# francescofugazzi/3dgsconverter

Measured on AMD Instinct MI355X. Metric: Msplats/sec SOR k=16, higher is better.
Workload: dtype f32 select / f64 finalize

## Files before the change

3dgsconverter_amd/_lib.py:

```python
from __future__ import annotations

import contextlib
import ctypes as C
import functools
import os
import threading
import time

import numpy as np

_HERE = os.path.dirname(os.path.abspath(__file__))
LIB_PATH = os.environ.get("GSX_LIB_PATH") or os.path.join(_HERE, "libgsx_hip.so")

KNN_AUTO, KNN_BRUTE, KNN_GRID, KNN_TREE = 0, 1, 2, 3
PROBE_ROOT_DIST2, PROBE_ROOT_DSQRT = 0, 1
PROBE_MEAN_NET, PROBE_MEAN_LIST, PROBE_MEAN_LE128, PROBE_MEAN_NP = 0, 1, 2, 3
T_SOR_KNN, T_SOR_BIN, T_SOR_FALLBACK, T_SOR_STATS, T_DENSITY, T_KMEANS_ASSIGN, T_KMEANS_UPDATE, T_QUANTIZE = range(8)
T_SLAB_PREP, T_SLAB_ROWS, T_SLAB_MEANS, T_SLAB_COLL = range(8, 12)


class GsxError(RuntimeError):
    """Raised for every failure of the HIP path (missing library, no GPU, HIP error)."""


# ... 115 lines not shown

DENSITY_OK, DENSITY_EMPTY, DENSITY_HOST = range(3)
SLAB_OK, SLAB_EMPTY, SLAB_NONFINITE, SLAB_SMALL_SHARD, SLAB_NO_STRUCTURE = range(5)
COMM_F32_MAX, COMM_F32_SUM, COMM_I64_SUM, COMM_F64_MAX, COMM_I64_MIN = range(5)

_P, _I64, _I, _D = C.c_void_p, C.c_int64, C.c_int, C.c_double
SIGNATURES = {
    "gsx_version": (C.c_char_p, []),
    "gsx_last_error": (C.c_char_p, []),
    "gsx_device_count": (_I, []),
    "gsx_device_uid": (_I, [_I, C.c_char_p, _I]),
    "gsx_ctx_create": (_I, [_I, C.POINTER(_P)]),
    "gsx_ctx_destroy": (None, [_P]),
    "gsx_ctx_set_stream": (_I, [_P, _P]),
    "gsx_ctx_own_stream": (_I, [_P]),
    "gsx_ctx_last_knn_algo": (_I, [_P]),
    "gsx_ctx_synchronize": (_I, [_P]),
    "gsx_ctx_check": (_I, [_P]),
    "gsx_ctx_set_timing": (_I, [_P, _I]),
    "gsx_ctx_reset_timing": (_I, [_P]),
    "gsx_ctx_get_timing": (_I, [_P, _I, C.POINTER(C.c_uint64), C.POINTER(_D)]),
    "gsx_ctx_set_param": (_I, [_P, C.c_char_p, _D]),
    "gsx_dev_malloc": (_I, [_P, C.c_size_t, C.POINTER(_P)]),
    "gsx_dev_free": (_I, [_P, _P]),
    "gsx_dev_upload": (_I, [_P, _P, _P, C.c_size_t]),
    "gsx_dev_download": (_I, [_P, _P, _P, C.c_size_t]),
    "gsx_dev_copy": (_I, [_P, _P, _P, C.c_size_t]),
    "gsx_dev_upload_async": (_I, [_P, _P, _P, C.c_size_t]),
    "gsx_dev_memset": (_I, [_P, _P, _I, C.c_size_t]),
    "gsx_fields_nonzero_dev": (_I, [_P, _P, _I64, _I64, _I, C.POINTER(C.c_uint64)]),
    "gsx_rows_repack_dev": (_I, [_P, _P, _I64, _I64, _P, _I64]),
    "gsx_host_pinned_alloc": (_I, [_P, C.c_size_t, C.POINTER(C.c_void_p)]),
    "gsx_host_pinned_free": (_I, [_P, _P]),
    "gsx_dev_upload_staged": (_I, [_P, _P, _P, C.c_size_t]),
    "gsx_dev_download_staged": (_I, [_P, _P, _P, C.c_size_t]),
    "gsx_host_gather_f32": (_I, [_P, _I64, _I64, C.POINTER(_I64), _I, _P]),
    "gsx_host_gather_columns_f32": (_I, [_P, _I64, _I64, C.POINTER(_I64), _I, _P]),
    "gsx_host_compact_rows": (_I, [_P, _I64, _I64, _P, _P, _I64, C.POINTER(_I64)]),
    "gsx_host_take_rows": (_I, [_P, _I64, _I64, _P, _I64, _P]),
    "gsx_host_zero_columns": (_I, [_P, _I64, _I64, C.POINTER(_I64), _I]),
    "gsx_host_append_columns": (_I, [_P, _I64, _I64, _P, _I64, _P, _I64]),
    "gsx_host_take_rows_append": (_I, [_P, _I64, _I64, _P, _I64, _P, _I64, _P, _I64]),
    "gsx_host_take_rows_shape": (_I, [_P, _I64, _I64, _P, _I64, _P, _I64, C.POINTER(_I64), _I, _P, _I64]),
    "gsx_rgb_from_sh": (_I, [_P, _I64, _P, _P]),
    "gsx_rgb_from_sh_dev": (_I, [_P, _P, _I64, _P, _P]),
    "gsx_rgb_from_sh_list": (_I, [_P, _I64, _P, _P, _I64, C.POINTER(_I64)]),
    "gsx_rgb_from_sh_list_dev": (_I, [_P, _P, _I64, _P, _P, _I64, _P]),
    "gsx_compact_rows_dev": (_I, [_P, _P, _P, _P, _I64, _P, _P, C.POINTER(_I64)]),
    "gsx_mask_bbox_dev": (_I, [_P, _P, _I64, _P, _P]),
    "gsx_mask_ge_dev": (_I, [_P, _P, _P, _I64, _D, _P]),
    "gsx_sor_knn_dev": (_I, [_P, _P, _P, _P, _I64, _I64, _I64, _I64, _I, _I, _P, C.POINTER(SorInfo)]),
    "gsx_sor_knn_share_dev": (_I, [_P, _P, _P, _P, _I64, _I64, _I, _I, _I, _I, _P, C.POINTER(SorInfo)]),
    "gsx_sor_debug_brick_plan": (_I, [_P, _P, _P, _P, _I64]),
    "gsx_sor_debug_work_queue": (_I, [_P, _P, _P, _P]),
    "gsx_sor_debug_wave_stamps": (_I, [_P, _I, _P, _I64, _P]),
    "gsx_knn_probe_root_dev": (_I, [_P, _P, _I64, _I, _P]),
    "gsx_knn_probe_mean_dev": (_I, [_P, _P, _I64, _I64, _I, _I, _I, _P]),
    "gsx_sor_stats_dev": (_I, [_P, _P, _I64, _D, _P]),
    "gsx_sor_mask_dev": (_I, [_P, _P, _I64, _P, _P]),
    "gsx_comm_unique_id": (_I, [_P]),
    "gsx_comm_init": (_I, [_P, _I, _I, _P]),
    "gsx_comm_destroy": (_I, [_P]),
    "gsx_comm_all_reduce": (_I, [_P, _P, _I64, _I]),
    "gsx_comm_all_gather": (_I, [_P, _P, _P, _I64]),
    "gsx_comm_all_to_all_v": (_I, [_P, _P, _P, _P, _P, _P, _P, _I]),
    "gsx_comm_all_to_all_segs": (_I, [_P, _P, _P, _I, _P, _P, _P, _P, _I]),
    "gsx_comm_abort": (_I, [_P]),
    "gsx_comm_transport": (_I, [_P]),
    "gsx_comm_rank": (_I, [_P, C.POINTER(_I), C.POINTER(_I)]),
    "gsx_comm_barrier": (_I, [_P]),
    "gsx_slab_plan": (_I, [_P, _I, _I, _I64, _I, _D, C.POINTER(SlabPlan)]),
    "gsx_sor_slab_step_dev": (_I, [_P, _P, _I64, _I, _D, _D, _P, C.POINTER(SlabStep)]),
    "gsx_slab_bbox_dev": (_I, [_P, _P, _P, _P, _I64, _I64, _P]),
    "gsx_slab_hist_dev": (_I, [_P, _P, _P, _P, _I64, _I64, _P, _P]),
    "gsx_slab_partition_dev": (_I, [_P, _P, _P, _P, _I64, _I64, _I, _I, C.c_float, C.c_float, _P, _I, _P, _P, _P, _P, _P]),
    "gsx_sor_knn_slab_dev": (_I, [_P, _P, _I64, _I64, _I, _P, _P]),
    "gsx_slab_certify_dev": (_I, [_P, _P, _I64, _I64, _P, C.c_float, C.c_float, _P]),
    "gsx_slab_unpermute_dev": (_I, [_P, _P, _P, _I64, _P]),
    "gsx_sor_piece_sums_dev": (_I, [_P, _P, _I64, _P, _P]),
    "gsx_sor_stats_from_pieces_dev": (_I, [_P, _P, _I64, _I64, _I, _D, _P]),
    "gsx_sor_filter": (_I, [_P, _P, _P, _I64, _I64, _I, _D, _I, _P, _P, _P, C.POINTER(SorInfo)]),
    "gsx_density_voxels": (_I, [_P, _P, _P, _I64, _I64, _D, _I64, _I64, C.POINTER(_I64), C.POINTER(_I64), _P, _P]),
    "gsx_density_mask": (_I, [_P, _P, _P, _I64, _I64, _D, _P, _I64, _P]),
    "gsx_kmeans_lloyd": (_I, [_P, _I64, _I, _I, _I, _P, _P, _P]),
    "gsx_quantize_sorted_codebook": (_I, [_P, _I64, _P, _I, _P]),
    "gsx_kmeans_pp": (_I, [_P, _I64, _I, _I, _P, _I, _P]),
    "gsx_kmeans_pp_dev": (_I, [_P, _P, _I64, _I, _I, _P, _I, _P]),
    "gsx_kmeans1d": (_I, [_P, _I64, _I, _I, _P, _P, _P]),
    "gsx_kmeans1d_dev": (_I, [_P, _P, _I64, _I, _I, _I, _P, _P, _P]),
    "gsx_lexsort3": (_I, [_P, _P, _P, _I64, _P]),
    "gsx_lexsort3_dev": (_I, [_P, _P, _P, _P, _I64, _I64, _P]),
    "gsx_sog_quats": (_I, [_P, _I64, _P]),
    "gsx_sog_positions": (_I, [_P, _I64, C.c_float, C.c_float, _P, _P]),
    "gsx_sog_positions_dev": (_I, [_P, _P, _I64, C.c_float, C.c_float, _P, _P]),
    "gsx_sog_alpha": (_I, [_P, _I64, _P, _P]),
    "gsx_sog_alpha_dev": (_I, [_P, _P, _I64, _P, _P]),
    "gsx_sog_quats_dev": (_I, [_P, _P, _I64, _P]),
    "gsx_sog_scan_dev": (_I, [_P, _P, C.POINTER(SogLayout), _I64, _P, C.POINTER(SogScan)]),
    "gsx_sog_extremes_dev": (_I, [_P, _P, _I64, _P, _P, _I, _P, _P]),
    "gsx_sog_order_dev": (_I, [_P, _P, _I64, _P]),
    "gsx_sog_gather_dev": (_I, [_P, _P, C.POINTER(SogLayout), _P, _I64, _I, _P, _P, _P, _P, _P, _P]),
    "gsx_sog_means_texels_dev": (_I, [_P, _P, _I64, _I64, _P, _P, _P, _P, _P, _P, _P, _I64, _P]),
    "gsx_sog_quats_texels_dev": (_I, [_P, _P, _I64, _I64, _P]),
    "gsx_sog_codes_texels_dev": (_I, [_P, _P, _I64, _I64, _P, _I, _P, _P, _P, _I64, _P]),
    "gsx_sog_labels_texels_dev": (_I, [_P, _P, _I64, _I64, _I64, _I, _P]),
    "gsx_gather_rows_dev": (_I, [_P, _P, _I, _P, _I64, _P]),
# ... 1853 lines not shown
        check(self.lib.gsx_ctx_synchronize(self.handle), "gsx_ctx_synchronize")

    def check(self):
        check(self.lib.gsx_ctx_check(self.handle), "gsx_ctx_check")

    def last_knn_algo(self) -> int:
        return int(self.lib.gsx_ctx_last_knn_algo(self.handle))

    def set_param(self, name: str, value: float):
        check(self.lib.gsx_ctx_set_param(self.handle, name.encode(), float(value)), "gsx_ctx_set_param")

    def set_timing(self, on: bool):
        check(self.lib.gsx_ctx_set_timing(self.handle, 1 if on else 0), "gsx_ctx_set_timing")

    def reset_timing(self):
        check(self.lib.gsx_ctx_reset_timing(self.handle), "gsx_ctx_reset_timing")

    def timing(self, slot: int):
        n = C.c_uint64()
        ms = C.c_double()
        check(self.lib.gsx_ctx_get_timing(self.handle, int(slot), C.byref(n), C.byref(ms)), "gsx_ctx_get_timing")
        return int(n.value), float(ms.value)

    def alloc(self, nbytes: int) -> DeviceArray:
        return DeviceArray(self, nbytes)

    def sor_knn(self, x: int, y: int, z: int, stride: int, n_ref: int, q_begin: int, q_count: int, k: int,
                mean_out: int, algo: int = KNN_AUTO, want_info: bool = False):
        info = SorInfo() if want_info else None
        check(self.lib.gsx_sor_knn_dev(self.handle, x, y, z, stride, n_ref, q_begin, q_count, int(k), int(algo),
                                       mean_out, C.byref(info) if want_info else None), "gsx_sor_knn_dev")
        return info.as_dict() if want_info else None

    def sor_knn_share(self, x: int, y: int, z: int, stride: int, n: int, k: int, share: int, nshares: int,
                      mean_out: int, algo: int = KNN_AUTO, want_info: bool = False):
        info = SorInfo() if want_info else None
        check(self.lib.gsx_sor_knn_share_dev(self.handle, x, y, z, stride, n, int(k), int(algo), int(share),
                                             int(nshares), mean_out, C.byref(info) if want_info else None),
              "gsx_sor_knn_share_dev")
        return info.as_dict() if want_info else None

    def debug_brick_plan(self, cap: int = 1 << 22):
        import numpy as np
        grid = (C.c_int32 * 8)()
        origin = (C.c_float * 4)()
        buf = np.zeros((cap, 2), np.uint32)
        check(self.lib.gsx_sor_debug_brick_plan(self.handle, grid, origin, buf.ctypes.data_as(C.c_void_p), cap),
              "gsx_sor_debug_brick_plan")
        m = min(int(grid[4]), cap) if grid[3] else 0
        runs = np.stack([buf[:m, 0], buf[:m, 1] & 0xffff, buf[:m, 1] >> 16], axis=1).astype(np.int64)
        return {"nx": int(grid[0]), "ny": int(grid[1]), "nz": int(grid[2]), "plan": int(grid[3]), "bricks": int(grid[4]),
                "origin": np.array(list(origin), np.float32), "runs": runs}

    def debug_work_queue(self):
        import numpy as np
        ctr = np.zeros((4, 8), np.uint32)
        items = np.zeros(4, np.int64)
        blocks = np.zeros(4, np.int32)
        check(self.lib.gsx_sor_debug_work_queue(self.handle, ctr.ctypes.data_as(C.c_void_p), items.ctypes.data_as(C.c_void_p),
                                                blocks.ctypes.data_as(C.c_void_p)), "gsx_sor_debug_work_queue")
        names = ("knn_brick", "knn_brick_extra", "knn_ring", "knn_ring_fast")
        return {nm: {"ctr": ctr[i].astype(np.int64), "items": int(items[i]), "blocks": int(blocks[i])} for i, nm in enumerate(names)}

    def debug_wave_stamps(self, kernel: int):
        import numpy as np
        cap = 1 << 14
        buf = np.zeros((cap, 16), np.uint64)
        count = C.c_int64()
        check(self.lib.gsx_sor_debug_wave_stamps(self.handle, int(kernel), buf.ctypes.data_as(C.c_void_p), cap, C.byref(count)),
              "gsx_sor_debug_wave_stamps")
        rec = buf[:min(cap, int(count.value))]
        return rec[rec[:, 14] == 1]

    def knn_probe_root(self, values: int, n: int, mode: int, out: int):
        check(self.lib.gsx_knn_probe_root_dev(self.handle, values, int(n), int(mode), out), "gsx_knn_probe_root_dev")

    def knn_probe_mean(self, d2: int, m: int, stride: int, k: int, form: int, cap: int, out: int):
        check(self.lib.gsx_knn_probe_mean_dev(self.handle, d2, int(m), int(stride), int(k), int(form), int(cap), out),
              "gsx_knn_probe_mean_dev")

    def sor_stats(self, mean_dists: int, n: int, threshold_factor: float, stats_out: int):
        check(self.lib.gsx_sor_stats_dev(self.handle, mean_dists, n, float(threshold_factor), stats_out),
              "gsx_sor_stats_dev")

    def sor_mask(self, mean_dists: int, n: int, threshold_ptr: int, mask_out: int):
        check(self.lib.gsx_sor_mask_dev(self.handle, mean_dists, n, threshold_ptr, mask_out), "gsx_sor_mask_dev")


class DeviceArena:

    def __init__(self, device: int = 0):
        self.device = int(device)
        self.closed = False
        self._ctxs = {}
        self._sides = {}
        self._bufs = {}
        self._pinned = {}
        self._leases = set()

    @staticmethod
    def group(name: str) -> str:
        return name.split("_", 1)[0]

    def _require(self, group: str, what: str):
        if group not in self._leases:
            raise RuntimeError("DeviceArena: %s used without holding the %r lease" % (what, group))
# ... 383 lines not shown
```

3dgsconverter_amd/csrc/api.hip:

```cpp
#include <algorithm>
#include <mutex>

#include "gsx_common.h"
#include "sor_grid_params.h"

namespace gsx {

static thread_local std::string g_err;

void set_error(const char *fmt, ...)
{
    char buf[1024];
    va_list ap;
    va_start(ap, fmt);
    vsnprintf(buf, sizeof(buf), fmt, ap);
    va_end(ap);
    g_err = buf;
}

int DevBuf::reserve(size_t bytes)
{
    if (bytes <= cap) return 0;
    if (p) {
        GSX_HIP(hipFree(p));
// ... 322 lines not shown

int gsx_sor_knn_dev(gsx_ctx *c, const float *x, const float *y, const float *z, int64_t stride, int64_t n_ref,
                    int64_t q_begin, int64_t q_count, int k, int algo, float *mean_out, gsx_sor_info *info)
{
    if (!c || !x || !y || !z || !mean_out) GSX_FAIL("gsx_sor_knn_dev: null argument");
    if (n_ref <= 0 || n_ref >= (1LL << 31) - 1024) GSX_FAIL("gsx_sor_knn_dev: n_ref=%lld out of range", (long long)n_ref);
    if (q_begin < 0 || q_count < 0 || q_begin + q_count > n_ref) GSX_FAIL("gsx_sor_knn_dev: query range out of bounds");
    if (k < 1 || k > 2047) GSX_FAIL("gsx_sor_knn_dev: k=%d not supported (1 <= k <= 2047)", k);
    if (stride < 1) GSX_FAIL("gsx_sor_knn_dev: bad stride");
    GSX_HIP(hipSetDevice(c->device));
    if (q_count == 0) return 0;
    if (algo == GSX_KNN_AUTO) algo = n_ref < c->brute_below ? GSX_KNN_BRUTE : GSX_KNN_GRID;
    if (k > 64) algo = GSX_KNN_GRID;
    if (algo == GSX_KNN_BRUTE) {
        GSX_CHECK(c->ws[0].packed.reserve(sizeof(float4) * (size_t)n_ref));
        GSX_CHECK(timing_begin(c, GSX_T_SOR_BIN));
        GSX_CHECK(launch_pack_points(c, x, y, z, stride, n_ref, c->ws[0].packed.as<float4>()));
        GSX_CHECK(timing_end(c, GSX_T_SOR_BIN));
        GSX_CHECK(timing_begin(c, GSX_T_SOR_KNN));
        GSX_CHECK(launch_knn_brute(c, c->ws[0].packed.as<float4>(), n_ref, q_begin, q_count, nullptr, nullptr, 0, k, mean_out));
        GSX_CHECK(timing_end(c, GSX_T_SOR_KNN));
        if (info) {
            memset(info, 0, sizeof(*info));
            info->algo = GSX_KNN_BRUTE;
            GSX_HIP(hipStreamSynchronize(c->stream));
        }
        return 0;
    }
    if (algo == GSX_KNN_GRID) return launch_knn_grid(c, x, y, z, stride, n_ref, q_begin, q_count, k, mean_out, info);
    if (algo == GSX_KNN_TREE) return launch_knn_tree(c, x, y, z, stride, n_ref, q_begin, q_count, k, mean_out, nullptr, info, INT32_MAX, 0, 1, false);
    GSX_FAIL("gsx_sor_knn_dev: unknown algo %d", algo);
}

int gsx_sor_debug_brick_plan(gsx_ctx *c, int32_t *grid, float *origin, uint32_t *list, int64_t cap)
{
    if (!c || !grid || !origin) GSX_FAIL("gsx_sor_debug_brick_plan: null argument");
    gsx::KnnWs &w = c->ws[0];
    if (!w.gridparams.p) GSX_FAIL("gsx_sor_debug_brick_plan: no grid KNN call has run on this context");
    GSX_HIP(hipSetDevice(c->device));
    gsx::GridParams h;
    GSX_HIP(hipMemcpyAsync(&h, w.gridparams.p, sizeof(h), hipMemcpyDeviceToHost, c->stream));
    GSX_HIP(hipStreamSynchronize(c->stream));
    const int32_t g[8] = {h.nx, h.ny, h.nz, h.plan, h.nbricks, 0, 0, 0};
    memcpy(grid, g, sizeof(g));
    const float o[4] = {h.ox, h.oy, h.oz, h.inv_h};
    memcpy(origin, o, sizeof(o));
    if (h.plan && list && w.bricklist.p) {
        const int64_t m = std::min<int64_t>(h.nbricks, cap);
        if (m > 0) GSX_HIP(hipMemcpy(list, w.bricklist.p, sizeof(uint32_t) * 2 * (size_t)m, hipMemcpyDeviceToHost));
    }
    return 0;
}

int gsx_sor_debug_work_queue(gsx_ctx *c, uint32_t *ctr, int64_t *items, int32_t *blocks)
{
    if (!c || !ctr || !items || !blocks) GSX_FAIL("gsx_sor_debug_work_queue: null argument");
    gsx::KnnWs &w = c->ws[0];
    if (!w.gridparams.p) GSX_FAIL("gsx_sor_debug_work_queue: no grid KNN call has run on this context");
    GSX_HIP(hipSetDevice(c->device));
    gsx::GridParams h;
    GSX_HIP(hipMemcpyAsync(&h, w.gridparams.p, sizeof(h), hipMemcpyDeviceToHost, c->stream));
    GSX_HIP(hipStreamSynchronize(c->stream));
    const unsigned *src[4] = {h.brick_ctr, h.extra_ctr, h.ring_ctr, h.ringf_ctr};
    for (int q = 0; q < 4; ++q)
        for (int y = 0; y < 8; ++y) ctr[q * 8 + y] = src[q][y * 32];
    items[0] = h.part_hi - h.part_lo;
    items[1] = h.extra_count;
    items[2] = c->ring_fast ? h.ring2_count : h.fail_count;
    items[3] = c->ring_fast ? h.fail_count : 0;
    for (int q = 0; q < 4; ++q) blocks[q] = c->wq_grid[q];
    return 0;
}

int gsx_sor_debug_wave_stamps(gsx_ctx *c, int kernel, uint64_t *out, int64_t cap, int64_t *count)
{
    if (!c || !out || !count || kernel < 0 || kernel > 1) GSX_FAIL("gsx_sor_debug_wave_stamps: bad arguments");
#ifdef GSX_WAVE_STAMPS
    gsx::KnnWs &w = c->ws[0];
    if (!w.wavestamps.p) GSX_FAIL("gsx_sor_debug_wave_stamps: no grid KNN call has run on this context");
    GSX_HIP(hipSetDevice(c->device));
    GSX_HIP(hipStreamSynchronize(c->stream));
    const int64_t slots = c->ws_cap;
    const int64_t m = std::min<int64_t>(slots, cap);
    if (m > 0)
        GSX_HIP(hipMemcpy(out, (const uint64_t *)w.wavestamps.p + (size_t)kernel * slots * gsx::WS_WORDS,
                          sizeof(uint64_t) * gsx::WS_WORDS * (size_t)m, hipMemcpyDeviceToHost));
    *count = slots;
    return 0;
#else
    (void)cap;
    GSX_FAIL("gsx_sor_debug_wave_stamps needs a diagnostic build of the library (-DGSX_WAVE_STAMPS)");
#endif
}

int gsx_sor_knn_share_dev(gsx_ctx *c, const float *x, const float *y, const float *z, int64_t stride, int64_t n,
                          int k, int algo, int share, int nshares, float *mean_out, gsx_sor_info *info)
{
    if (!c || !x || !y || !z || !mean_out) GSX_FAIL("gsx_sor_knn_share_dev: null argument");
    if (nshares < 1 || share < 0 || share >= nshares) GSX_FAIL("gsx_sor_knn_share_dev: share %d of %d", share, nshares);
    if (n <= 0 || n >= (1LL << 31) - 1024) GSX_FAIL("gsx_sor_knn_share_dev: n=%lld out of range", (long long)n);
    if (k < 1 || k > 64) GSX_FAIL("gsx_sor_knn_share_dev: k=%d not supported (1 <= k <= 64)", k);
    if (stride < 1) GSX_FAIL("gsx_sor_knn_share_dev: bad stride");
    GSX_HIP(hipSetDevice(c->device));
    GSX_HIP(hipMemsetAsync(mean_out, 0, sizeof(float) * (size_t)n, c->stream));
    if (algo == GSX_KNN_AUTO) algo = n < c->brute_below ? GSX_KNN_BRUTE : GSX_KNN_GRID;
    if (algo == GSX_KNN_BRUTE) {
// ... 423 lines not shown
```

3dgsconverter_amd/csrc/gsx_common.h:

```cpp
#pragma once

#include <hip/hip_runtime.h>

#include <cstdarg>
#include <cstdint>
#include <cstdio>
#include <cstring>
#include <string>
#include <vector>

#include "../../include/gsx_hip.h"

namespace gsx {

constexpr int WAVE = 64;

void set_error(const char *fmt, ...);

#define GSX_HIP(call)                                                                         \
    do {                                                                                      \
        hipError_t e__ = (call);                                                              \
        if (e__ != hipSuccess) {                                                              \
            gsx::set_error("%s failed: %s (%s:%d)", #call, hipGetErrorString(e__), __FILE__,  \
                           __LINE__);                                                         \
            return 1;                                                                         \
        }                                                                                     \
    } while (0)

#define GSX_CHECK(expr)            \
    do {                           \
        int r__ = (expr);          \
        if (r__ != 0) return r__;  \
    } while (0)

#define GSX_FAIL(...)                \
    do {                             \
        gsx::set_error(__VA_ARGS__); \
        return 1;                    \
    } while (0)

struct DevBuf {
    void *p = nullptr;
    size_t cap = 0;
    int reserve(size_t bytes);
    void release();
    template <class T>
    T *as() const { return reinterpret_cast<T *>(p); }
};

constexpr int KNN_MAX_LEVELS = 5;
struct KnnWs {
    DevBuf packed;
    DevBuf qsorted;
    DevBuf bucketpts;
    DevBuf bkcnt;
    DevBuf tilecnt;
    DevBuf tileoff;
    DevBuf cellstart;
    DevBuf qcellstart;
    DevBuf gridparams;
    DevBuf bboxpart;
    DevBuf faillist;
    DevBuf extraitems;
    DevBuf finestart;
    DevBuf bricklist;
    DevBuf bundleoff;
    DevBuf wavestamps;
    DevBuf deferred;
    DevBuf cellflag;
    DevBuf subxyz;
    DevBuf submap;
    DevBuf submean;
    DevBuf subkth;
    DevBuf heavylist;
    DevBuf heavypart;
    DevBuf probe;
    uint64_t refined_total = 0;
    void release_all()
    {
        DevBuf *all[] = {&packed, &qsorted, &bucketpts, &bkcnt, &tilecnt, &tileoff, &cellstart, &qcellstart, &gridparams, &bboxpart,
                         &faillist, &extraitems, &finestart, &bricklist, &bundleoff, &wavestamps, &deferred, &cellflag, &subxyz, &submap, &submean, &subkth,
                         &heavylist, &heavypart, &probe};
        for (auto b : all) b->release();
    }
};

constexpr int GSX_TREE_UNSUITABLE = 2;

struct TreeWs {
    DevBuf keys[2];
    DevBuf vals[2];
    DevBuf refs;
    DevBuf samples;
    DevBuf blockboxes;
    DevBuf flags;
    DevBuf tilecnt, tileoff;
    DevBuf leafstart;
    DevBuf leafbl;
    DevBuf faillist;
    DevBuf failbound;
    DevBuf bboxpart;
    DevBuf params;
    DevBuf temp;
    void release_all()
    {
        DevBuf *all[] = {&keys[0], &keys[1], &vals[0], &vals[1], &refs, &samples, &blockboxes, &flags, &tilecnt, &tileoff, &leafstart, &leafbl,
                         &faillist, &failbound, &bboxpart, &params, &temp};
        for (auto b : all) b->release();
    }
};

struct SlabWs {
    DevBuf plan_in;
    DevBuf hist;
    DevBuf small;
    DevBuf send;
    DevBuf send_src;
    DevBuf slab;
    DevBuf md_slab;
    DevBuf kth;
    DevBuf ret;
    DevBuf md;
    DevBuf md_stats;
    DevBuf pieces, allpieces, packed;
    DevBuf mask;
    void *host = nullptr;
    size_t host_cap = 0;
    void release_all()
    {
        DevBuf *all[] = {&plan_in, &hist, &small, &send, &send_src, &slab, &md_slab, &kth, &ret, &md, &md_stats, &pieces, &allpieces, &packed, &mask};
// ... 77 lines not shown
```

3dgsconverter_amd/csrc/sor_grid.hip:

```cpp
#include <algorithm>
#include <chrono>
#include <cmath>
#include <cstdlib>
#include <type_traits>
#include <unordered_map>
#include <vector>

#include "gsx_common.h"
#include "knn_common.h"
#include "knn_mfma.h"
#include "sor_grid_params.h"

namespace gsx {


constexpr int MAX_DIM = 1024;
constexpr int MAX_BUCKETS = 4096;
constexpr int MAX_BUCKET_CELLS = 4096;
#ifndef GSX_BUCKET_POINTS
#define GSX_BUCKET_POINTS 4096
#endif
constexpr int BUCKET_POINTS = GSX_BUCKET_POINTS;
#ifndef GSX_BIN_TILE
#define GSX_BIN_TILE 8192
// ... 529 lines not shown
#pragma unroll
        for (int k = 0; k < SCATTER_THREADS / 64; ++k) {
            const unsigned q = wsum[k];
            if (k < w) base += q;
            tot += q;
        }
        __syncthreads();
        const unsigned ex = carry + base + inc - v;
        if (i < nb) tab[i] = ex;
        gb[u] -= ex;
        carry += tot;
    }
    __syncthreads();
#pragma unroll
    for (int u = 0; u < SCATTER_PPT; ++u) {
        const int i = lo + u * SCATTER_THREADS + (int)threadIdx.x;
        if (i < hi)
            stage[tab[bk[u]] + rk[u]] = make_float4(px[u], py[u], pz[u],
                                                    __uint_as_float((unsigned)(first + i) | (i >= ref_only_from ? 0x80000000u : 0u)));
    }
    __syncthreads();
#pragma unroll
    for (int u = 0; u < BPT; ++u) {
        const int i = u * SCATTER_THREADS + (int)threadIdx.x;
        if (i < nb) tab[i] = gb[u];
    }
    __syncthreads();
#pragma unroll
    for (int u = 0; u < SCATTER_PPT; ++u) {
        const int j = u * SCATTER_THREADS + (int)threadIdx.x;
        if (j < hi - lo) {
            const float4 r = stage[j];
            out[tab[bucket_of(g, cell_coord(r.y, g.oy, g.inv_h, g.ny), cell_coord(r.z, g.oz, g.inv_h, g.nz))] + j] = r;
        }
    }
}

#ifndef GSX_SORT_THREADS
#define GSX_SORT_THREADS 512
#endif
#ifndef GSX_SORT_PPT
#define GSX_SORT_PPT 16
#endif
constexpr int SORT_THREADS = GSX_SORT_THREADS;
constexpr int SORT_PPT = GSX_SORT_PPT;
constexpr unsigned SORT_CAP = SORT_THREADS * SORT_PPT;

__device__ __forceinline__ int quarter_coord(float v, float o, float inv_h, int dim)
{
    int c = (int)((v - o) * (4.0f * inv_h));
    return min(max(c, 0), 4 * dim - 1);
}

template <bool FINE>
__global__ __launch_bounds__(SORT_THREADS) void bucket_sort_kernel(const GridParams *__restrict__ gp,
                                                          const unsigned *__restrict__ bk_start,
                                                          const float4 *__restrict__ in, float4 *__restrict__ out,
                                                          unsigned *__restrict__ cell_start, unsigned big_limit,
                                                          unsigned *__restrict__ fine_start)
{
    constexpr int SUB = FINE ? 4 : 1;
    __shared__ unsigned cnt[SUB * MAX_BUCKET_CELLS];
    __shared__ unsigned wsum[SORT_THREADS / 64];
    const GridParams g = *gp;
    const int b = blockIdx.x;
    if (g.bad_input || b >= g.bk_count) return;
    const int ncell = g.bk_cells;
    const int cells = SUB * ncell;
    const unsigned s0 = bk_start[b], s1 = bk_start[b + 1];
    if (b == g.bk_count - 1 && threadIdx.x == 0) {
        cell_start[(size_t)g.bk_count * ncell] = s1;
        if (FINE) fine_start[(size_t)g.bk_count * cells] = s1;
    }
    if (s1 - s0 > big_limit) return;
    const int by = b % g.bk_ny, bz = b / g.bk_ny;
    for (int i = threadIdx.x; i < cells; i += SORT_THREADS) cnt[i] = 0;
    __syncthreads();
    auto local_cell = [&](const float4 p) {
        const int cx = FINE ? quarter_coord(p.x, g.ox, g.inv_h, g.nx) : cell_coord(p.x, g.ox, g.inv_h, g.nx);
        const int cy = cell_coord(p.y, g.oy, g.inv_h, g.ny);
        const int cz = cell_coord(p.z, g.oz, g.inv_h, g.nz);
        return ((cz - bz * g.bk_g) * g.bk_g + (cy - by * g.bk_g)) * (SUB * g.nx) + cx;
    };
    const bool fits = s1 - s0 <= SORT_CAP;
    float4 p[SORT_PPT];
    int cell[SORT_PPT];
    unsigned rk[SORT_PPT];
    if (fits) {
#pragma unroll
        for (int u = 0; u < SORT_PPT; ++u) p[u] = in[min(s0 + u * SORT_THREADS + threadIdx.x, s1 - 1)];
#pragma unroll
        for (int u = 0; u < SORT_PPT; ++u) {
            cell[u] = local_cell(p[u]);
            rk[u] = s0 + u * SORT_THREADS + threadIdx.x < s1 ? atomicAdd(&cnt[cell[u]], 1u) : 0u;
        }
    } else {
        for (unsigned i = s0 + threadIdx.x; i < s1; i += SORT_THREADS) atomicAdd(&cnt[local_cell(in[i])], 1u);
    }
    __syncthreads();
    const int seg = (cells + SORT_THREADS - 1) / SORT_THREADS;
    const int c0 = min(cells, (int)threadIdx.x * seg), c1 = min(cells, c0 + seg);
    unsigned sum = 0;
    for (int c = c0; c < c1; ++c) sum += cnt[c];
    unsigned inc = sum;
#pragma unroll
    for (int off = 1; off < 64; off <<= 1) {
        unsigned o = __shfl_up(inc, off);
        if ((int)(threadIdx.x & 63) >= off) inc += o;
    }
    const int wv = threadIdx.x >> 6;
    if ((threadIdx.x & 63) == 63) wsum[wv] = inc;
    __syncthreads();
    unsigned run = inc - sum;
    for (int i = 0; i < wv; ++i) run += wsum[i];
    __syncthreads();
    for (int c = c0; c < c1; ++c) {
        const unsigned v = cnt[c];
        cnt[c] = run;
        run += v;
    }
    __syncthreads();
    unsigned *cs = cell_start + (size_t)b * ncell;
    for (int i = threadIdx.x; i < ncell; i += SORT_THREADS) cs[i] = s0 + cnt[SUB * i];
    if (FINE) {
        unsigned *fs = fine_start + (size_t)b * cells;
        for (int i = threadIdx.x; i < cells; i += SORT_THREADS) fs[i] = s0 + cnt[i];
    }
    if (fits) {
#pragma unroll
        for (int u = 0; u < SORT_PPT; ++u)
            if (s0 + u * SORT_THREADS + threadIdx.x < s1) out[s0 + cnt[cell[u]] + rk[u]] = p[u];
    } else {
        __syncthreads();
        for (unsigned i = s0 + threadIdx.x; i < s1; i += SORT_THREADS) {
            const float4 q = in[i];
            out[s0 + atomicAdd(&cnt[local_cell(q)], 1u)] = q;
        }
    }
}

constexpr unsigned BIG_BUCKET = 32768;
constexpr int BIG_CHUNK = 8192;

__device__ __forceinline__ int bucket_containing(const unsigned *bk_start, int nb, unsigned pos)
{
    int lo = 0, hi = nb;
    while (hi - lo > 1) {
        const int mid = (lo + hi) >> 1;
        if (bk_start[mid] <= pos) lo = mid; else hi = mid;
    }
    return lo;
}

template <bool SCATTER>
__global__ __launch_bounds__(256) void big_bucket_kernel(const GridParams *__restrict__ gp, const unsigned *__restrict__ bk_start,
                                                         int n, const float4 *__restrict__ in, float4 *__restrict__ out,
                                                         unsigned *cell_start ,
                                                         unsigned *cursor )
{
    __shared__ unsigned cnt[MAX_BUCKET_CELLS];
    __shared__ unsigned base[SCATTER ? MAX_BUCKET_CELLS : 1];
    const GridParams g = *gp;
    if (g.bad_input) return;
    const unsigned lo = (unsigned)blockIdx.x * BIG_CHUNK;
    if (lo >= (unsigned)n) return;
    const unsigned hi = min((unsigned)n, lo + BIG_CHUNK);
    const int cells = g.bk_cells;
    for (int b = bucket_containing(bk_start, g.bk_count, lo); b < g.bk_count; ++b) {
        const unsigned s0 = bk_start[b], s1 = bk_start[b + 1];
        if (s0 >= hi) break;
        if (s1 - s0 <= BIG_BUCKET) continue;
        const unsigned p0 = max(lo, s0), p1 = min(hi, s1);
        const int by = b % g.bk_ny, bz = b / g.bk_ny;
        auto local_cell = [&](const float4 p) {
            const int cx = cell_coord(p.x, g.ox, g.inv_h, g.nx);
            const int cy = cell_coord(p.y, g.oy, g.inv_h, g.ny);
            const int cz = cell_coord(p.z, g.oz, g.inv_h, g.nz);
            return ((cz - bz * g.bk_g) * g.bk_g + (cy - by * g.bk_g)) * g.nx + cx;
        };
        for (int i = threadIdx.x; i < cells; i += 256) cnt[i] = 0;
        __syncthreads();
        for (unsigned i = p0 + threadIdx.x; i < p1; i += 256) atomicAdd(&cnt[local_cell(in[i])], 1u);
        __syncthreads();
        unsigned *gc = (SCATTER ? cursor : cell_start) + (size_t)b * cells;
// ... 1874 lines not shown
        const int ws_cap = ctx->num_cu * 8 * (BRICK_THREADS / 64);
        const size_t ws_bytes = sizeof(unsigned long long) * 2 * (size_t)ws_cap * WS_WORDS;
        GSX_CHECK(w.wavestamps.reserve(ws_bytes));
        GSX_HIP(hipMemsetAsync(w.wavestamps.p, 0, ws_bytes, ctx->stream));
        gpa.stamps = w.wavestamps.as<unsigned long long>();
        gpa.stamps_cap = ws_cap;
        ctx->ws_cap = ws_cap;
    }
#endif
    const bool adaptive_at_bbox = adaptive;
    if (sk && sk->box.b7)
        hipLaunchKernelGGL(grid_params_known_box_kernel, dim3(1), dim3(64), 0, ctx->stream, sk->box, w.bboxpart.as<float>(), gpa);
    else
        hipLaunchKernelGGL(bbox_partial_kernel, dim3(bbox_blocks), dim3(256), 0, ctx->stream, x, y, z, stride, (int)n_ref,
                           w.bboxpart.as<float>(), gpa);
    GSX_HIP(hipGetLastError());
    if (adaptive) GSX_CHECK(w.qcellstart.reserve(sizeof(unsigned) * (size_t)(cap + 1)));
    bool tree_ok = (adaptive || (slab && ctx->adaptive)) && ctx->tree && level == 0 && kk <= 65 && n_ref > k;
    bool hist_done = false;
    if (tree_ok) {
        GSX_CHECK(bin_hist(ctx, w, x, y, z, stride, 0, n_ref, gp));
        static thread_local std::vector<unsigned> starts(MAX_BUCKETS + 1);
        GSX_HIP(hipMemcpyAsync(starts.data(), w.bkcnt.as<unsigned>() + MAX_BUCKETS, sizeof(unsigned) * (MAX_BUCKETS + 1), hipMemcpyDeviceToHost, ctx->stream));
        GSX_HIP(hipStreamSynchronize(ctx->stream));
        unsigned mx = 0, nonzero = 0;
        for (int b = 0; b < MAX_BUCKETS; ++b) {
            const unsigned c = starts[b + 1] >= starts[b] ? starts[b + 1] - starts[b] : 0u;
            mx = std::max(mx, c);
            nonzero += c > 0;
        }
        hist_done = true;
        if (nonzero > 0 && (double)mx > 3.0 * (double)n_ref / (double)nonzero) {
            GSX_CHECK(timing_end(ctx, GSX_T_SOR_BIN));
            if (getenv("GSX_TRACE_LEVELS"))
                fprintf(stderr, "[gsx] level 0: fullest bucket %u of %lld points in %u buckets -> tree path\n", mx, (long long)n_ref, nonzero);
            const int rc = launch_knn_tree(ctx, x, y, z, stride, n_ref, q_begin, q_count, k, mean_out, kth_out, info,
                                           slab ? ref_only_from : INT32_MAX, share, nshares, true);
            if (rc != GSX_TREE_UNSUITABLE) return rc;
            tree_ok = false;
            ctx->last_knn_algo = GSX_KNN_GRID;
            GSX_CHECK(timing_begin(ctx, GSX_T_SOR_BIN));
        }
        if (nonzero > 0 && (double)mx <= 1.5 * (double)n_ref / (double)nonzero && nshares == 1) adaptive = false;
    }
    if (adaptive_at_bbox && !adaptive) {
        GSX_HIP(hipMemsetAsync(&gp->defer_words, 0, sizeof(int), ctx->stream));
        GSX_HIP(hipMemsetAsync(&gp->heavy_limit, 0, sizeof(int), ctx->stream));
    }
    if (plan && adaptive) {
        plan = false;
        GSX_HIP(hipMemsetAsync(&gp->plan, 0, sizeof(int), ctx->stream));
    }
    unsigned *fstart = plan ? w.finestart.as<unsigned>() : nullptr;
    GSX_CHECK(bin_points(ctx, w, x, y, z, stride, 0, n_ref, gp, rstart, refs, cap, adaptive ? w.qcellstart.as<unsigned>() : nullptr,
                         slab ? ref_only_from : INT32_MAX, hist_done, fstart));
    if (plan) {
        unsigned *bcnt = w.bundleoff.as<unsigned>(), *boff = bcnt + (size_t)(MAX_DIM / 2) * (MAX_DIM / 2);
        const int pblocks = ctx->num_cu * 4;
        hipLaunchKernelGGL(brick_plan_kernel<false>, dim3(pblocks), dim3(64 * PLAN_WAVES), 0, ctx->stream, gp, fstart, bcnt, boff,
                           w.bricklist.as<uint2>());
        hipLaunchKernelGGL(brick_plan_kernel<true>, dim3(pblocks), dim3(64 * PLAN_WAVES), 0, ctx->stream, gp, fstart, bcnt, boff,
                           w.bricklist.as<uint2>());
        GSX_HIP(hipGetLastError());
    }
    const float4 *qpts = refs;
    const unsigned *qstart = rstart;
    if (!all) {
        GSX_CHECK(bin_points(ctx, w, x, y, z, stride, q_begin, q_count, gp, w.qcellstart.as<unsigned>(),
                             w.qsorted.as<float4>()));
        qpts = w.qsorted.as<float4>();
        qstart = w.qcellstart.as<unsigned>();
    }
    GSX_CHECK(timing_end(ctx, GSX_T_SOR_BIN));

    BrickLaunch a{gp, refs, rstart, qpts, qstart, k, q_begin, mean_out, kth_out, w.faillist.as<unsigned>(),
                  w.faillist.as<unsigned>() + std::max<int64_t>(q_count, 1),
                  w.extraitems.as<uint2>(), w.deferred.as<unsigned>(), w.heavylist.as<unsigned>(), q_count, n_ref,
                  plan ? w.finestart.as<unsigned>() : nullptr, plan ? w.bricklist.as<uint2>() : nullptr};
    if (anyk) {
        GSX_CHECK(timing_begin(ctx, GSX_T_SOR_KNN));
        const int blocks = (int)std::max<int64_t>(1, std::min<int64_t>((q_count + 3) / 4, (int64_t)ctx->num_cu * 2));
        hipLaunchKernelGGL(knn_anyk_kernel, dim3(blocks), dim3(BRICK_THREADS), 0, ctx->stream, gp, refs, rstart, qpts, (int)q_count, k,
                           (int)q_begin, mean_out, kth_out);
        GSX_HIP(hipGetLastError());
        GSX_CHECK(timing_end(ctx, GSX_T_SOR_KNN));
        if (info) {
            GridParams h2;
            GSX_HIP(hipMemcpyAsync(&h2, gp, sizeof(GridParams), hipMemcpyDeviceToHost, ctx->stream));
            GSX_HIP(hipStreamSynchronize(ctx->stream));
            info->algo = GSX_KNN_GRID;
            info->grid_dim[0] = h2.nx;
            info->grid_dim[1] = h2.ny;
            info->grid_dim[2] = h2.nz;
            info->cell_size = h2.h;
            info->n_cells = (int64_t)h2.nx * h2.ny * h2.nz;
            info->n_bricks = 0;
            info->n_fallback = q_count;
            info->n_exhaustive = h2.exhaustive_count;
            info->n_deferred_bricks = 0;
            info->n_refined = 0;
        }
        return 0;
    }
    GSX_CHECK(dispatch_bricks(ctx, a, mfma_ok, ctx->phase2_net != 0));

    const bool trace = getenv("GSX_TRACE_LEVELS") != nullptr;
// ... 254 lines not shown
```

include/gsx_hip.h:

```cpp
#ifndef GSX_HIP_H
#define GSX_HIP_H

#include <stddef.h>
#include <stdint.h>

#ifdef __cplusplus
extern "C" {
#endif

typedef struct gsx_ctx gsx_ctx;

enum {
    GSX_KNN_AUTO = 0,
    GSX_KNN_BRUTE = 1,
    GSX_KNN_GRID = 2,
    GSX_KNN_TREE = 3
};

enum {
    GSX_T_SOR_KNN = 0,
    GSX_T_SOR_BIN = 1,
    GSX_T_SOR_FALLBACK = 2,
    GSX_T_SOR_STATS = 3,
    GSX_T_DENSITY = 4,
// ... 34 lines not shown
int  gsx_ctx_set_timing(gsx_ctx *ctx, int enable);
int  gsx_ctx_reset_timing(gsx_ctx *ctx);
int  gsx_ctx_get_timing(gsx_ctx *ctx, int slot, uint64_t *launches, double *total_ms);
int  gsx_ctx_set_param(gsx_ctx *ctx, const char *name, double value);

int gsx_dev_malloc(gsx_ctx *ctx, size_t bytes, void **dptr);
int gsx_dev_free(gsx_ctx *ctx, void *dptr);
int gsx_host_pinned_alloc(gsx_ctx *ctx, size_t bytes, void **hptr);
int gsx_host_pinned_free(gsx_ctx *ctx, void *hptr);
int gsx_dev_upload(gsx_ctx *ctx, void *dst_dev, const void *src_host, size_t bytes);
int gsx_dev_download(gsx_ctx *ctx, void *dst_host, const void *src_dev, size_t bytes);
int gsx_dev_copy(gsx_ctx *ctx, void *dst_dev, const void *src_dev, size_t bytes);
int gsx_dev_upload_async(gsx_ctx *ctx, void *dst_dev, const void *src_host, size_t bytes);
int gsx_dev_memset(gsx_ctx *ctx, void *dst_dev, int value, size_t bytes);
int gsx_dev_upload_staged(gsx_ctx *ctx, void *dst_dev, const void *src_host, size_t bytes);
int gsx_dev_download_staged(gsx_ctx *ctx, void *dst_host, const void *src_dev, size_t bytes);

int gsx_host_gather_f32(const void *rows, int64_t row_bytes, int64_t n, const int64_t *offsets,
                        int ncols, float *out);
int gsx_host_gather_columns_f32(const void *rows, int64_t row_bytes, int64_t n, const int64_t *offsets,
                                int ncols, float *out);
int gsx_host_compact_rows(const void *rows, int64_t row_bytes, int64_t n, const uint8_t *mask,
                          void *out, int64_t out_rows, int64_t *n_out);
int gsx_host_take_rows(const void *rows, int64_t row_bytes, int64_t n, const uint32_t *idx, int64_t n_idx, void *out);

int gsx_compact_rows_dev(gsx_ctx *ctx, const float *rows_dev, const uint32_t *orig_dev, const uint8_t *mask_dev, int64_t n,
                         float *rows_out_dev, uint32_t *orig_out_dev, int64_t *n_out);

int gsx_rgb_from_sh(const float *f_dc, int64_t n, uint8_t *out, uint8_t *uncertain_out);
int gsx_rgb_from_sh_dev(gsx_ctx *ctx, const float *f_dc_dev, int64_t n, uint8_t *out_dev, uint8_t *uncertain_dev);
int gsx_rgb_from_sh_list(const float *f_dc, int64_t n, uint8_t *out, uint32_t *list_out, int64_t cap, int64_t *count_out);
int gsx_rgb_from_sh_list_dev(gsx_ctx *ctx, const float *f_dc_dev, int64_t n, uint8_t *out_dev, uint32_t *list_dev, int64_t cap,
                             uint32_t *count_dev);
int gsx_host_zero_columns(void *rows, int64_t row_bytes, int64_t n, const int64_t *offsets, int ncols);
int gsx_host_append_columns(const void *rows, int64_t row_bytes, int64_t n, const uint8_t *extra, int64_t extra_bytes,
                            void *out, int64_t out_row_bytes);
int gsx_host_take_rows_append(const void *rows, int64_t row_bytes, int64_t n, const uint32_t *idx, int64_t n_idx,
                              const uint8_t *extra, int64_t extra_bytes, void *out, int64_t out_row_bytes);
int gsx_host_take_rows_shape(const void *rows, int64_t row_bytes, int64_t n, const uint32_t *idx, int64_t n_idx,
                             const uint8_t *extra, int64_t extra_bytes, const int64_t *zero_offsets, int nzero, void *out,
                             int64_t out_row_bytes);

int gsx_mask_bbox_dev(gsx_ctx *ctx, const float *rows_dev, int64_t n, const double *bounds6, uint8_t *mask_dev);
int gsx_mask_ge_dev(gsx_ctx *ctx, const float *vals_dev, const uint32_t *orig_dev, int64_t n, double threshold,
                    uint8_t *mask_dev);

int gsx_sor_knn_dev(gsx_ctx *ctx, const float *x, const float *y, const float *z, int64_t stride,
                    int64_t n_ref, int64_t q_begin, int64_t q_count, int k, int algo,
                    float *mean_out_dev, gsx_sor_info *info );
int gsx_sor_knn_share_dev(gsx_ctx *ctx, const float *x, const float *y, const float *z, int64_t stride,
                          int64_t n, int k, int algo, int share, int nshares, float *mean_out_dev,
                          gsx_sor_info *info );
int gsx_sor_debug_brick_plan(gsx_ctx *ctx, int32_t *grid, float *origin, uint32_t *list, int64_t cap);
int gsx_sor_debug_work_queue(gsx_ctx *ctx, uint32_t *ctr, int64_t *items, int32_t *blocks);
int gsx_sor_debug_wave_stamps(gsx_ctx *ctx, int kernel, uint64_t *out, int64_t cap, int64_t *count);
enum { GSX_PROBE_ROOT_DIST2 = 0, GSX_PROBE_ROOT_DSQRT = 1 };
int gsx_knn_probe_root_dev(gsx_ctx *ctx, const double *in_dev, int64_t n, int mode, double *out_dev);
enum { GSX_PROBE_MEAN_NET = 0, GSX_PROBE_MEAN_LIST = 1, GSX_PROBE_MEAN_LE128 = 2, GSX_PROBE_MEAN_NP = 3 };
int gsx_knn_probe_mean_dev(gsx_ctx *ctx, const double *d2_dev, int64_t m, int64_t stride, int k, int form, int cap,
                           float *out_dev);
int gsx_sor_stats_dev(gsx_ctx *ctx, const float *mean_dists_dev, int64_t n, double threshold_factor,
                      float *stats_dev);
int gsx_sor_mask_dev(gsx_ctx *ctx, const float *mean_dists_dev, int64_t n, const float *threshold_dev,
                     uint8_t *mask_out_dev);

enum { GSX_COMM_F32_MAX = 0, GSX_COMM_F32_SUM = 1, GSX_COMM_I64_SUM = 2, GSX_COMM_F64_MAX = 3, GSX_COMM_I64_MIN = 4 };
int gsx_comm_unique_id(void *out128);
int gsx_comm_init(gsx_ctx *ctx, int rank, int world, const void *id128);
int gsx_comm_destroy(gsx_ctx *ctx);
int gsx_comm_abort(gsx_ctx *ctx);
int gsx_comm_transport(gsx_ctx *ctx);
int gsx_comm_rank(gsx_ctx *ctx, int *rank_out, int *world_out);
int gsx_comm_barrier(gsx_ctx *ctx);
int gsx_comm_all_reduce(gsx_ctx *ctx, void *buf_dev, int64_t count, int kind);
int gsx_comm_all_gather(gsx_ctx *ctx, const void *send_dev, void *recv_dev, int64_t bytes_per_rank);
int gsx_comm_all_to_all_v(gsx_ctx *ctx, const void *send_dev, const int64_t *send_off, const int64_t *send_cnt,
                          void *recv_dev, const int64_t *recv_off, const int64_t *recv_cnt, int elem_bytes);
int gsx_comm_all_to_all_segs(gsx_ctx *ctx, const void *send_dev, void *recv_dev, int nseg, const int64_t *send_off,
                             const int64_t *send_cnt, const int64_t *recv_off, const int64_t *recv_cnt, int elem_bytes);

enum { GSX_SLAB_OK = 0, GSX_SLAB_EMPTY = 1, GSX_SLAB_NONFINITE = 2, GSX_SLAB_SMALL_SHARD = 3, GSX_SLAB_NO_STRUCTURE = 4 };
typedef struct gsx_slab_plan_t {
    int32_t status, world, rank, axis, halo_bins;
    float   lo, hi;
    float   plane_lo, plane_hi;
    int32_t cut[17];
    int64_t n_local, n_total, n_own, n_halo, n_send, halo_total;
    int64_t sizes[16];
    int64_t own_cnt[16], halo_cnt[16], own_off[16], halo_off[16];
    int64_t in_own[16], in_halo[16], r_own_off[16], r_halo_off[16];
} gsx_slab_plan_t;
typedef struct gsx_slab_step_t {
    int32_t status;
    gsx_slab_plan_t plan;
    const uint8_t *mask_dev;
    const float   *mean_dists_dev;
    const float   *stats_dev;
    const int64_t *uncertain_dev;
} gsx_slab_step_t;
int gsx_slab_plan(const uint32_t *words, int world, int rank, int64_t n_local, int k, double halo_cells, gsx_slab_plan_t *out);
int gsx_sor_slab_step_dev(gsx_ctx *ctx, const float *rows_dev, int64_t n_local, int k, double threshold_factor,
                          double halo_cells, uint8_t *mask_out_dev , gsx_slab_step_t *out);

int gsx_slab_bbox_dev(gsx_ctx *ctx, const float *x, const float *y, const float *z, int64_t stride, int64_t n,
                      float *out7_dev);
int gsx_slab_hist_dev(gsx_ctx *ctx, const float *x, const float *y, const float *z, int64_t stride, int64_t n,
// ... 298 lines not shown
```

Baseline: 5961.

## Stage bucket-sort scatter through LDS for coalesced writes and skip empty rounds

The bucket sort kernel now writes each point to its final rank inside a shared-memory stage buffer, then copies the stage out to global memory in contiguous runs, replacing the scattered per-point global stores. The per-cell counters are placed inside the same LDS allocation. Load and count rounds are unrolled in groups of four and stop early when the bucket holds fewer points. Launch bounds gain a minimum-blocks hint. The cost is extra syncthreads and a much larger LDS footprint per block, which may lower occupancy. A debug entry point that dumps the sorted cells is also added.

```diff
diff --git a/3dgsconverter_amd/_lib.py b/3dgsconverter_amd/_lib.py
--- a/3dgsconverter_amd/_lib.py
+++ b/3dgsconverter_amd/_lib.py
@@ -191,6 +191,7 @@
     "gsx_sor_knn_dev": (_I, [_P, _P, _P, _P, _I64, _I64, _I64, _I64, _I, _I, _P, C.POINTER(SorInfo)]),
     "gsx_sor_knn_share_dev": (_I, [_P, _P, _P, _P, _I64, _I64, _I, _I, _I, _I, _P, C.POINTER(SorInfo)]),
     "gsx_sor_debug_brick_plan": (_I, [_P, _P, _P, _P, _I64]),
+    "gsx_sor_debug_cells": (_I, [_P, _P, _P, _P, _I64, _P, _I64, _P, _I64]),
     "gsx_sor_debug_work_queue": (_I, [_P, _P, _P, _P]),
     "gsx_sor_debug_wave_stamps": (_I, [_P, _I, _P, _I64, _P]),
     "gsx_knn_probe_root_dev": (_I, [_P, _P, _I64, _I, _P]),
@@ -2150,6 +2151,24 @@
         return {"nx": int(grid[0]), "ny": int(grid[1]), "nz": int(grid[2]), "plan": int(grid[3]), "bricks": int(grid[4]),
                 "origin": np.array(list(origin), np.float32), "runs": runs}
 
+    def debug_cells(self):
+        import numpy as np
+        grid = (C.c_int32 * 12)()
+        origin = (C.c_float * 4)()
+        check(self.lib.gsx_sor_debug_cells(self.handle, grid, origin, None, 0, None, 0, None, 0), "gsx_sor_debug_cells")
+        names = ("nx", "ny", "nz", "bk_g", "bk_ny", "bk_nz", "bk_count", "bk_cells", "ncells", "n")
+        out = {nm: int(grid[i]) for i, nm in enumerate(names)}
+        n, ncells, fine = out["n"], out["ncells"], bool(grid[10])
+        rec = np.zeros((n, 4), np.uint32)
+        cs = np.zeros(ncells + 1, np.uint32)
+        fs = np.zeros(4 * ncells + 1, np.uint32) if fine else None
+        check(self.lib.gsx_sor_debug_cells(self.handle, grid, origin, rec.ctypes.data_as(C.c_void_p), n,
+                                           cs.ctypes.data_as(C.c_void_p), len(cs),
+                                           fs.ctypes.data_as(C.c_void_p) if fine else None, len(fs) if fine else 0),
+              "gsx_sor_debug_cells")
+        out.update(origin=np.array(list(origin), np.float32), records=rec, cell_start=cs, fine_start=fs)
+        return out
+
     def debug_work_queue(self):
         import numpy as np
         ctr = np.zeros((4, 8), np.uint32)
diff --git a/3dgsconverter_amd/csrc/api.hip b/3dgsconverter_amd/csrc/api.hip
--- a/3dgsconverter_amd/csrc/api.hip
+++ b/3dgsconverter_amd/csrc/api.hip
@@ -398,6 +398,35 @@
     return 0;
 }
 
+int gsx_sor_debug_cells(gsx_ctx *c, int32_t *grid, float *origin, float *records, int64_t rec_cap, uint32_t *cell_start,
+                        int64_t cell_cap, uint32_t *fine_start, int64_t fine_cap)
+{
+    if (!c || !grid || !origin) GSX_FAIL("gsx_sor_debug_cells: null argument");
+    gsx::KnnWs &w = c->ws[0];
+    if (!w.gridparams.p || !w.packed.p || !w.cellstart.p || w.sorted_n <= 0 || c->last_knn_algo != GSX_KNN_GRID)
+        GSX_FAIL("gsx_sor_debug_cells: the context's last KNN call did not run on the grid");
+    GSX_HIP(hipSetDevice(c->device));
+    gsx::GridParams h;
+    GSX_HIP(hipMemcpyAsync(&h, w.gridparams.p, sizeof(h), hipMemcpyDeviceToHost, c->stream));
+    GSX_HIP(hipStreamSynchronize(c->stream));
+    if (h.bad_input) GSX_FAIL("gsx_sor_debug_cells: the last call met non-finite coordinates, nothing was sorted");
+    const int64_t n = w.sorted_n, ncells = h.ncells;
+    const bool fine = w.fine_sorted && w.finestart.p;
+    if (ncells <= 0 || sizeof(uint32_t) * (size_t)(ncells + 1) > w.cellstart.cap || sizeof(float) * 4 * (size_t)n > w.packed.cap ||
+        (fine && sizeof(uint32_t) * (size_t)(4 * ncells + 1) > w.finestart.cap))
+        GSX_FAIL("gsx_sor_debug_cells: the grid of the last call does not match the context's tables");
+    const int32_t g[12] = {h.nx, h.ny, h.nz, h.bk_g, h.bk_ny, h.bk_nz, h.bk_count, h.bk_cells, (int32_t)ncells, (int32_t)n, fine ? 1 : 0, 0};
+    memcpy(grid, g, sizeof(g));
+    const float o[4] = {h.ox, h.oy, h.oz, h.inv_h};
+    memcpy(origin, o, sizeof(o));
+    if (records && rec_cap >= n) GSX_HIP(hipMemcpy(records, w.packed.p, sizeof(float) * 4 * (size_t)n, hipMemcpyDeviceToHost));
+    if (cell_start && cell_cap >= ncells + 1)
+        GSX_HIP(hipMemcpy(cell_start, w.cellstart.p, sizeof(uint32_t) * (size_t)(ncells + 1), hipMemcpyDeviceToHost));
+    if (fine && fine_start && fine_cap >= 4 * ncells + 1)
+        GSX_HIP(hipMemcpy(fine_start, w.finestart.p, sizeof(uint32_t) * (size_t)(4 * ncells + 1), hipMemcpyDeviceToHost));
+    return 0;
+}
+
 int gsx_sor_debug_work_queue(gsx_ctx *c, uint32_t *ctr, int64_t *items, int32_t *blocks)
 {
     if (!c || !ctr || !items || !blocks) GSX_FAIL("gsx_sor_debug_work_queue: null argument");
diff --git a/3dgsconverter_amd/csrc/gsx_common.h b/3dgsconverter_amd/csrc/gsx_common.h
--- a/3dgsconverter_amd/csrc/gsx_common.h
+++ b/3dgsconverter_amd/csrc/gsx_common.h
@@ -76,6 +76,8 @@
     DevBuf heavypart;
     DevBuf probe;
     uint64_t refined_total = 0;
+    int64_t sorted_n = 0;
+    bool fine_sorted = false;
     void release_all()
     {
         DevBuf *all[] = {&packed, &qsorted, &bucketpts, &bkcnt, &tilecnt, &tileoff, &cellstart, &qcellstart, &gridparams, &bboxpart,
diff --git a/3dgsconverter_amd/csrc/sor_grid.hip b/3dgsconverter_amd/csrc/sor_grid.hip
--- a/3dgsconverter_amd/csrc/sor_grid.hip
+++ b/3dgsconverter_amd/csrc/sor_grid.hip
@@ -605,15 +605,21 @@
     return min(max(c, 0), 4 * dim - 1);
 }
 
+constexpr int SORT_STAGE = 4096;
+constexpr int SORT_GROUP = 4;
+static_assert(SORT_PPT % SORT_GROUP == 0, "the rounds of a thread are unrolled in whole groups");
+
 template <bool FINE>
-__global__ __launch_bounds__(SORT_THREADS) void bucket_sort_kernel(const GridParams *__restrict__ gp,
+__global__ __launch_bounds__(SORT_THREADS, SORT_THREADS / 128) void bucket_sort_kernel(const GridParams *__restrict__ gp,
                                                           const unsigned *__restrict__ bk_start,
                                                           const float4 *__restrict__ in, float4 *__restrict__ out,
                                                           unsigned *__restrict__ cell_start, unsigned big_limit,
                                                           unsigned *__restrict__ fine_start)
 {
     constexpr int SUB = FINE ? 4 : 1;
-    __shared__ unsigned cnt[SUB * MAX_BUCKET_CELLS];
+    static_assert(SUB * MAX_BUCKET_CELLS * sizeof(unsigned) <= SORT_STAGE * sizeof(float4), "the counters live inside the stage's bytes");
+    __shared__ float4 stage[SORT_STAGE];
+    unsigned *cnt = reinterpret_cast<unsigned *>(stage);
     __shared__ unsigned wsum[SORT_THREADS / 64];
     const GridParams g = *gp;
     const int b = blockIdx.x;
@@ -635,17 +641,26 @@
         const int cz = cell_coord(p.z, g.oz, g.inv_h, g.nz);
         return ((cz - bz * g.bk_g) * g.bk_g + (cy - by * g.bk_g)) * (SUB * g.nx) + cx;
     };
-    const bool fits = s1 - s0 <= SORT_CAP;
+    const unsigned npts = s1 - s0;
+    const bool fits = npts <= SORT_CAP;
     float4 p[SORT_PPT];
     int cell[SORT_PPT];
     unsigned rk[SORT_PPT];
     if (fits) {
 #pragma unroll
-        for (int u = 0; u < SORT_PPT; ++u) p[u] = in[min(s0 + u * SORT_THREADS + threadIdx.x, s1 - 1)];
-#pragma unroll
-        for (int u = 0; u < SORT_PPT; ++u) {
-            cell[u] = local_cell(p[u]);
-            rk[u] = s0 + u * SORT_THREADS + threadIdx.x < s1 ? atomicAdd(&cnt[cell[u]], 1u) : 0u;
+        for (int gr = 0; gr < SORT_PPT; gr += SORT_GROUP) {
+            if ((unsigned)gr * SORT_THREADS >= npts) break;
+#pragma unroll
+            for (int u = gr; u < gr + SORT_GROUP; ++u) p[u] = in[min(s0 + u * SORT_THREADS + threadIdx.x, s1 - 1)];
+        }
+#pragma unroll
+        for (int gr = 0; gr < SORT_PPT; gr += SORT_GROUP) {
+            if ((unsigned)gr * SORT_THREADS >= npts) break;
+#pragma unroll
+            for (int u = gr; u < gr + SORT_GROUP; ++u) {
+                cell[u] = local_cell(p[u]);
+                rk[u] = u * SORT_THREADS + threadIdx.x < npts ? atomicAdd(&cnt[cell[u]], 1u) : 0u;
+            }
         }
     } else {
         for (unsigned i = s0 + threadIdx.x; i < s1; i += SORT_THREADS) atomicAdd(&cnt[local_cell(in[i])], 1u);
@@ -681,8 +696,28 @@
     }
     if (fits) {
 #pragma unroll
-        for (int u = 0; u < SORT_PPT; ++u)
-            if (s0 + u * SORT_THREADS + threadIdx.x < s1) out[s0 + cnt[cell[u]] + rk[u]] = p[u];
+        for (int gr = 0; gr < SORT_PPT; gr += SORT_GROUP) {
+            if ((unsigned)gr * SORT_THREADS >= npts) break;
+#pragma unroll
+            for (int u = gr; u < gr + SORT_GROUP; ++u)
+                rk[u] = u * SORT_THREADS + threadIdx.x < npts ? cnt[cell[u]] + rk[u] : 0xffffffffu;
+        }
+        const int lead = (int)(s0 & 7u);
+        for (unsigned w0 = 0; w0 < npts; w0 += SORT_STAGE) {
+            __syncthreads();
+#pragma unroll
+            for (int gr = 0; gr < SORT_PPT; gr += SORT_GROUP) {
+                if ((unsigned)gr * SORT_THREADS >= npts) break;
+#pragma unroll
+                for (int u = gr; u < gr + SORT_GROUP; ++u)
+                    if (rk[u] - w0 < (unsigned)SORT_STAGE) stage[rk[u] - w0] = p[u];
+            }
+            __syncthreads();
+            const int len = (int)min(npts - w0, (unsigned)SORT_STAGE);
+            float4 *dst = out + s0 + w0;
+            for (int j = (int)threadIdx.x - lead; j < len; j += SORT_THREADS)
+                if (j >= 0) dst[j] = stage[j];
+        }
     } else {
         __syncthreads();
         for (unsigned i = s0 + threadIdx.x; i < s1; i += SORT_THREADS) {
@@ -2663,6 +2698,8 @@
         GSX_HIP(hipMemsetAsync(&gp->plan, 0, sizeof(int), ctx->stream));
     }
     unsigned *fstart = plan ? w.finestart.as<unsigned>() : nullptr;
+    w.sorted_n = n_ref;
+    w.fine_sorted = fstart != nullptr;
     GSX_CHECK(bin_points(ctx, w, x, y, z, stride, 0, n_ref, gp, rstart, refs, cap, adaptive ? w.qcellstart.as<unsigned>() : nullptr,
                          slab ? ref_only_from : INT32_MAX, hist_done, fstart));
     if (plan) {
diff --git a/include/gsx_hip.h b/include/gsx_hip.h
--- a/include/gsx_hip.h
+++ b/include/gsx_hip.h
@@ -110,6 +110,8 @@
                           int64_t n, int k, int algo, int share, int nshares, float *mean_out_dev,
                           gsx_sor_info *info );
 int gsx_sor_debug_brick_plan(gsx_ctx *ctx, int32_t *grid, float *origin, uint32_t *list, int64_t cap);
+int gsx_sor_debug_cells(gsx_ctx *ctx, int32_t *grid, float *origin, float *records, int64_t rec_cap, uint32_t *cell_start,
+                        int64_t cell_cap, uint32_t *fine_start, int64_t fine_cap);
 int gsx_sor_debug_work_queue(gsx_ctx *ctx, uint32_t *ctr, int64_t *items, int32_t *blocks);
 int gsx_sor_debug_wave_stamps(gsx_ctx *ctx, int kernel, uint64_t *out, int64_t cap, int64_t *count);
 enum { GSX_PROBE_ROOT_DIST2 = 0, GSX_PROBE_ROOT_DSQRT = 1 };
```

Result: no change. 6009, median of 6 (+0.8%).
